# spyglass-search/memex

Hardware: AMD Instinct MI355X
Metric: queries/sec, exact cosine top-10 (recall@10 = 1.0) on 10M x 384-d f32 (higher is better)
Workload: dtype f32 corpus; int8 MFMA filter (exact integer sums, measured-residual certificate) -> f32 rescoring -> f64 DistCosine on the survivors (results bit-identical to all-f64)

## Files before the change

### memex_amd/csrc/index.hip

```cpp
#include <dlfcn.h>
#include <sys/stat.h>
#include <unistd.h>

#include <algorithm>
#include <atomic>
#include <cmath>
#include <condition_variable>
#include <cstdlib>
#include <chrono>
#include <ctime>
#include <cstring>
#include <deque>
#include <map>
#include <memory>
#include <mutex>
#include <string>
#include <thread>
#include <vector>

#include "index_kernels.h"
#include "mx_common.h"
#include "mx_debug.h"
#include "shard_pool.h"

// ... 124 lines not shown
    uint64_t plain_bf16_rows = 0;
    uint64_t demoted_at_rows = 0;
    float *tsc = nullptr;
    float *amean = nullptr;
    float *mean = nullptr;
    float *msum = nullptr;
    bool centred = false;
    bool compressed = false;
    bool raw_ingest = false;
    float *xs = nullptr, *ss = nullptr;
    uint64_t xs_rows = 0;
    uint64_t n = 0, cap = 0;
    IdMap idmap{0, 0, 1, 0};
    uint32_t *flags = nullptr;
    uint64_t wild_rows = 0;
    uint32_t *zero_rows = nullptr;
    uint64_t n_zero = 0;
    uint32_t *wild_list = nullptr;
    uint64_t n_wild = 0;
    int mode = MX_SEARCH_AUTO;
    bool profiling = false;
    int n_cu = 0, nwg = 0;
    bool scan8_pair = true;
    Scratch s;
    mx_index_stats stats{};
    hipEvent_t ev0 = nullptr, ev1 = nullptr, ev_wait = nullptr;
    double wait_ema_us[4] = {0.0, 0.0, 0.0, 0.0};
    uint64_t *dead = nullptr;
    std::vector<uint64_t> dead_h;
    uint64_t n_dead = 0;
    std::vector<uint64_t> dead_log;
    uint64_t disk_dead = 0;
    uint64_t gen = 0;
    bool failed = false;
    uint64_t *filt = nullptr;
    size_t filt_words = 0;
    uint64_t *filt_ranges = nullptr;
    size_t filt_ranges_cap = 0;
    uint32_t *subset_rows = nullptr;
    bool last_subset = false;
    std::string disk_dir;
    uint64_t disk_rows = 0;
    off_t disk_size = 0;
    struct timespec disk_mtime {};
    std::vector<mx_index *> shards;
    uint64_t block_rows = 0;
// ... 463 lines not shown
    idx->n += n;
    if (idx->filter_auto && idx->xh && !idx->filter_i8 && idx->demoted_at_rows && idx->n >= 2 * idx->demoted_at_rows &&
        idx->ds <= kAutoI8MaxDim) {
        const std::string keep = last_error_slot();
        if (build_filter_copy(idx, true) == MX_OK) {
            idx->demoted_at_rows = 0;
            idx->stats.filter_promotions += 1;
        } else {
            idx->demoted_at_rows = idx->n;
            last_error_slot() = keep;
        }
    }
    if (idx->xh && !idx->filter_i8 && !idx->compressed && !idx->centred && idx->kc <= kMaxKC && idx->n >= 256 &&
        idx->n >= 2 * std::max<uint64_t>(idx->plain_bf16_rows, 128) && !(idx->filter_auto && idx->demoted_at_rows)) {
        const std::string keep = last_error_slot();
        if (build_filter_copy(idx, false) != MX_OK) {
            idx->plain_bf16_rows = idx->n;
            last_error_slot() = keep;
        }
    }
    return MX_OK;
}

uint32_t sample_stride(uint64_t full_tiles, int nwg, int k, bool filt8, int ds, bool centred8 = false) {
    (void)centred8;
    double div = !filt8 ? 64.0 : ds <= 512 ? 16.0 : ds <= 768 ? 8.0 : 4.0;
    if (const int dv = debug_flag("sample_div", 0); dv >= 2 && dv <= 4096) div = (double)dv;
    const double f = std::min(0.5, std::max(1.0 / div, (double)k / 640.0));
    const uint64_t target = std::max<uint64_t>((uint64_t)nwg, (uint64_t)((double)full_tiles * f));
    return (uint32_t)std::max<uint64_t>(1, full_tiles / std::max<uint64_t>(target, 1));
}

constexpr size_t kExactKeepBytes = 256ull << 20;

int run_exact(mx_index *idx, const std::vector<int> &qs, int k, uint64_t *d_ids, float *d_scores, float *d_dists,
              int32_t *d_nfound, const uint64_t *mask, uint64_t n_live) {
    if (qs.empty()) return MX_OK;
    int gcap = qs.size() <= 4 ? 4 : qs.size() <= 8 ? 8 : qs.size() <= 16 ? 16 : kExactGroup;
    int rc = ensure_exact(idx, k, &gcap);
    if (rc != MX_OK) return rc;
    Scratch &s = idx->s;
    for (size_t g0 = 0; g0 < qs.size(); g0 += (size_t)gcap) {
        ExactGroup grp{};
        grp.n = (int)std::min<size_t>((size_t)gcap, qs.size() - g0);
        for (int j = 0; j < grp.n; ++j) grp.q[j] = qs[g0 + j];
        MX_HIP(launch_exact_group(idx->stream, k, idx->ds, idx->compressed ? nullptr : idx->x, idx->xh, idx->n, idx->idmap, s.qpad,
                                  s.qnorm2, grp, s.exact_scratch, d_ids, d_scores, d_dists, d_nfound, mask, n_live));
    }
    return MX_OK;
}

int build_filter_copy(mx_index *idx, bool i8) {
    DevBuf nh, nts, nec, nam;
// ... 326 lines not shown
        const uint64_t ts0 = filt ? fr.front().first / trows : 0, ts1 = filt ? (fr.back().second + trows - 1) / trows : tiles;
        const uint64_t full1 = std::min(ts1, full);
        ScanParams p;
        p.x = idx->x;
        p.xh = idx->xh;
        p.scale = idx->scale;
        p.qfrag = s.qfrag;
        p.theta = s.theta;
        p.n_rows = idx->n;
        p.ds = (uint32_t)idx->ds;
        p.wave_mask = (1u << ((B + 31) / 32)) - 1u;
        p.lane_rec = s.lane_rec;
        p.lane_tile = s.lane_tile;
        p.lane_cnt = s.lane_cnt;
        p.lane_max = s.lane_max;
        p.overflow = s.overflow;
        p.tscale = idx->tsc;
        p.qscale = s.qscale;
        p.qa = s.qa;
        p.qb = s.qb;
        p.amean = centred ? idx->amean : nullptr;
        p.qmean = s.qmean;
        p.dead = mask;
        auto scan = [&](bool collect) {
            if (filt8) return launch_scan8(st, idx->kc, collect, nwg, p, pair ? Scan8Geom::kPair : x2 ? Scan8Geom::k512 : Scan8Geom::k256);
            if (wide) return launch_scan16w(st, idx->kc, collect, idx->nwg, p);
            return idx->xh ? launch_scan16(st, idx->kc, collect, idx->nwg, p) : launch_scan(st, idx->kc, collect, idx->nwg, p);
        };
        auto collect = [&](bool first) -> int {
            p.tile_begin = (uint32_t)ts0;
            p.tile_end = (uint32_t)ts1;
            p.tile_stride = 1;
            if (first && idx->profiling) MX_HIP(hipEventRecord(idx->ev0, st));
            MX_HIP(scan(true));
            if (first && idx->profiling) {
                MX_HIP(hipEventRecord(idx->ev1, st));
                timed = true;
            }
            if (first) {
                idx->stats.scan_launches += 1;
                idx->stats.scan_bytes += (ts1 - ts0) * trows * idx->ds * (filt8 ? 1ull : idx->xh ? 2ull : 4ull);
            }
            return MX_OK;
        };
        if (ts1 - ts0 > 2ull * idx->nwg) {
            p.tile_begin = (uint32_t)ts0;
            p.tile_end = (uint32_t)full1;
            p.tile_stride = sample_stride(full1 - ts0, nwg, k, filt8, idx->ds, centred8);
            MX_HIP(scan(false));
            MX_HIP(launch_theta(st, B, k, nwg, s.lane_max, s.qa, !filt8, s.theta));
        }
        if ((rc = collect(true)) != MX_OK) return rc;
        if ((rc = finish_and_wait()) != MX_OK) return rc;
        if (timed) {
            float ms = 0.f;
            MX_HIP(hipEventElapsedTime(&ms, idx->ev0, idx->ev1));
            idx->stats.scan_ms += ms;
            timed = false;
        }
        if (s.host_sum[2]) return fail(MX_EINVAL, "a query contains non-finite values");
        idx->stats.candidates += s.host_sum[1];
        if (s.host_sum[0]) {
            if ((rc = fetch_flags()) != MX_OK) return rc;
            int retry = 0;
            for (int b = 0; b < B; ++b) {
                if (h_ovf[b] == 1) ++retry;
                else if (h_ovf[b] >= 2) exact.push_back(b);
            }
            if (filt8 && !filt) idx->i8_retry_batches += 1;
            const bool habitual = filt8 && idx->i8_batches >= 8 && idx->i8_retry_batches * 4 > idx->i8_batches;
            if (filt8 && !filt && idx->filter_auto && ((size_t)(retry + (int)exact.size()) * 16 > (size_t)std::max(B, 16) || habitual)) {
                if (!idx->centred && idx->kc <= kMaxKC && idx->n >= 256) {
// ... 1005 lines not shown
        if (g_scan_setup_err == hipSuccess) g_scan_setup_err = range_setup();
    });
    if (g_scan_setup_err != hipSuccess)
        return fail(MX_EDEVICE, "scan kernel setup failed: %s (is this a gfx950 device?)", hipGetErrorString(g_scan_setup_err));
    std::unique_ptr<mx_index> idx(new mx_index());
    idx->key = k;
    idx->dim = dim;
    idx->ds = (int)round_up((uint64_t)dim, dim > kMaxKC * kChunkFloats ? 2 * kChunkFloats : kChunkFloats);
    idx->kc = idx->ds / kChunkFloats;
    {
        const char *fk = getenv("MEMEX_HIP_FILTER");
        idx->filter_auto = !(fk && fk[0]);
        idx->filter_i8 = idx->filter_auto ? idx->ds <= kAutoI8MaxDim : (fk[0] == 'i' || fk[0] == '8');
    }
    idx->device = device;
    hipDeviceProp_t prop;
    MX_HIP(hipGetDeviceProperties(&prop, device));
    idx->n_cu = prop.multiProcessorCount;
    idx->nwg = std::max(1, std::min(idx->n_cu, kMaxScanCUs));
    {
        const char *pv = getenv("MEMEX_HIP_SCAN8_PAIR");
        idx->scan8_pair = !(pv && pv[0] == '0');
    }
    MX_HIP(hipStreamCreateWithFlags(&idx->stream, hipStreamNonBlocking));
    MX_HIP(hipEventCreate(&idx->ev0));
    MX_HIP(hipEventCreate(&idx->ev1));
    MX_HIP(hipEventCreateWithFlags(&idx->ev_wait, hipEventDisableTiming));
    MX_HIP(hipMalloc(&idx->flags, 6 * sizeof(uint32_t)));
    MX_HIP(hipMemset(idx->flags, 0, 6 * sizeof(uint32_t)));
    MX_HIP(hipMalloc(&idx->zero_rows, kZeroCap * sizeof(uint32_t)));
    MX_HIP(hipMalloc(&idx->wild_list, kWildCap * sizeof(uint32_t)));
    if (device < kMaxDevices) {
        std::lock_guard<std::mutex> lk(g_lanes[device].mu);
        g_lanes[device].open_indexes += 1;
        idx->pooled = true;
    }
    *out = idx.release();
    return MX_OK;
}

bool row_removed(const mx_index *t, uint64_t r) {
    return t->dead && (r >> 6) < t->dead_h.size() && ((t->dead_h[r >> 6] >> (r & 63)) & 1ull);
}
bool global_removed(const mx_index *idx, uint64_t r) {
    if (!idx->composite()) return row_removed(idx, r);
    const uint64_t R = idx->block_rows, G = idx->shards.size(), b = r / R;
// ... 181 lines not shown
    return release_capacity(idx);
}

int compact_composite(mx_index *idx) {
    const uint64_t R = idx->block_rows, G = idx->shards.size(), total = idx->total;
    std::unique_ptr<mx_index> fresh(new mx_index());
    fresh->dim = idx->dim;
    fresh->block_rows = R;
    auto drop_fresh = [&] {
        for (mx_index *sh : fresh->shards) free_index(sh);
        fresh->shards.clear();
    };
    for (uint64_t g = 0; g < G; ++g) {
        mx_index *old = idx->shards[g], *sh = nullptr;
        int rc = open_plain("", idx->dim, old->device, &sh);
        if (rc != MX_OK) {
            drop_fresh();
            return rc;
        }
        sh->idmap = old->idmap;
        sh->mode = old->mode;
        sh->profiling = old->profiling;
        sh->scan8_pair = old->scan8_pair;
        sh->want_filter = old->want_filter;
        sh->filter_i8 = old->filter_i8;
        sh->filter_auto = old->filter_auto;
        sh->compressed = old->compressed;
        sh->raw_ingest = old->compressed;
        fresh->shards.push_back(sh);
    }
    const uint64_t chunk = std::max<uint64_t>(kTile8Rows, (32ull << 20) / ((uint64_t)idx->dim * 4));
    std::vector<float> buf((size_t)std::min<uint64_t>(chunk, std::max<uint64_t>(total, 1)) * idx->dim), tmpv;
    int rc = MX_OK;
    for (uint64_t r0 = 0; r0 < total && rc == MX_OK; r0 += chunk) {
        const uint64_t m = std::min(chunk, total - r0);
        rc = fetch_rows(idx, r0, m, buf.data(), tmpv);
        uint64_t k = 0;
        for (uint64_t i = 0; i < m && rc == MX_OK; ++i) {
            if (global_removed(idx, r0 + i)) continue;
            if (k != i) memmove(buf.data() + k * idx->dim, buf.data() + i * idx->dim, (size_t)idx->dim * sizeof(float));
            ++k;
        }
        if (rc == MX_OK && k) rc = composite_add(fresh.get(), buf.data(), k, nullptr, false);
    }
    for (mx_index *sh : fresh->shards) sh->raw_ingest = false;
    if (rc != MX_OK) {
// ... 1119 lines not shown
```

### memex_amd/csrc/index_kernels.h

```cpp
#pragma once
#include <hip/hip_runtime.h>

#include <cstdint>

namespace mx {

constexpr int kScanThreads = 512;
constexpr int kScanWaves = 8;
constexpr int kTileRows = 32;
constexpr int kChunkFloats = 128;
constexpr int kSlotBytes = kTileRows * kChunkFloats * 4;
constexpr int kNumSlots = 8;
constexpr int kPrefetch = 8;
constexpr int kScaleRing = 16;
constexpr int kScanLdsBytes = kNumSlots * kSlotBytes + 2 * kTileRows * (kChunkFloats * 2 + 16) + kScaleRing * kTileRows * 4;
constexpr int kMaxKC = 6;

constexpr int kSlot16Bytes = kTileRows * kChunkFloats * 2;
constexpr int kRing16 = 16;
constexpr int kMeanRing16 = 32;
constexpr int kScan16LdsBytes = kRing16 * kSlot16Bytes + kMeanRing16 * 256 + 1024;
constexpr int kMaxKC16 = 12;
constexpr int kWideBatch = 128;
constexpr int kScan16WideLdsBytes = kRing16 * kSlot16Bytes + 4 * 64 * 16 * 4;
// ... 29 lines not shown
struct ScanParams {
    const float *x;
    const void *xh;
    const float *scale;
    const void *qfrag;
    const float *theta;
    uint64_t n_rows;
    uint32_t tile_begin;
    uint32_t tile_end;
    uint32_t tile_stride;
    uint32_t ds;
    uint32_t wave_mask = 0xff;
    float *lane_rec;
    uint32_t *lane_tile;
    uint32_t *lane_cnt;
    float *lane_max;
    uint32_t *overflow;
    const float *tscale = nullptr;
    const float *qscale = nullptr;
    const float *qa = nullptr, *qb = nullptr;
    const float *amean = nullptr;
    const float *qmean = nullptr;
    const uint64_t *dead = nullptr;
};

__device__ __forceinline__ uint32_t lane_dead16(uint32_t half, uint32_t h) {
    const uint32_t w = half >> (4u * h);
    return (w & 0xfu) | ((w >> 4) & 0xf0u) | ((w >> 8) & 0xf00u) | ((w >> 12) & 0xf000u);
}
__device__ __forceinline__ uint32_t dead_half(const uint64_t *dead, uint32_t t) { return (uint32_t)(dead[t >> 1] >> (32u * (t & 1u))); }

hipError_t scan_setup();
hipError_t scan16_setup();
hipError_t launch_scan(hipStream_t s, int kc, bool collect, int nwg, const ScanParams &p);
hipError_t launch_scan16(hipStream_t s, int kc, bool collect, int nwg, const ScanParams &p);
constexpr int kTile8Rows = 64;
constexpr int kTscaleFloats = 8;
constexpr float kMinStep8 = 1.0f / 32768.0f;
constexpr int kScaleRing8 = 32;
constexpr int kScale8Entry = 512;
constexpr int kScan8LdsBytes = kRing16 * kSlot16Bytes + kScaleRing8 * kScale8Entry + 256;
constexpr int kScan8PairWaves = 4;
constexpr int kScan8PairRing = 8;
constexpr int kScan8PairScaleRing = 16;
constexpr int kScan8PairEntry = 256;
constexpr int kScan8PairLdsBytes = kScan8PairRing * kSlot16Bytes + kScan8PairScaleRing * kScan8PairEntry;
static_assert(2 * kScan8PairLdsBytes <= 160 * 1024, "two workgroups of the pair form must fit one CU's LDS");
enum class Scan8Geom {
    k256,
    k512,
    kPair,
};
hipError_t scan8_setup();
hipError_t launch_scan8(hipStream_t s, int kc, bool collect, int nwg, const ScanParams &p, Scan8Geom geom = Scan8Geom::k256);
hipError_t launch_shadow8(hipStream_t s, const float *x, const float *scale, int ds, uint32_t half0, uint32_t half1,
                          uint64_t row_hi, void *x8, float *tscale, uint32_t *ec_max, const float *mean = nullptr,
                          float *amean = nullptr, uint32_t *rc_max = nullptr);
hipError_t scan16w_setup();
hipError_t launch_scan16w(hipStream_t s, int kc, bool collect, int nwg, const ScanParams &p);

hipError_t launch_shadow(hipStream_t s, const float *x, const float *scale, int ds, uint32_t tile0, uint32_t tile1,
                         void *xh, uint32_t *ec_max, uint32_t src_tile0 = 0, uint64_t row_lo = 0, uint64_t row_hi = ~0ull,
                         const float *mean = nullptr, float *amean = nullptr);
hipError_t launch_mean_dir(hipStream_t s, const float *x, const float *scale, uint64_t n, int ds, float *msum, float *mean);
hipError_t launch_unshadow(hipStream_t s, const void *xh, int ds, int d, uint64_t row0, uint64_t n, float *out);

hipError_t launch_ingest(hipStream_t s, const float *src, uint64_t n, int d, float *x, float *scale,
                         uint64_t first, int ds, uint32_t *flags, int raw, uint32_t *zero_rows, uint32_t *wild_rows, uint64_t row_base);

hipError_t launch_prep_queries(hipStream_t s, const float *q, int B, int d, int ds, void *qfrag,
                               float *qpad, double *qnorm2, float *theta, float *e1, const uint32_t *ec_max,
                               uint32_t *overflow, uint32_t *flags, float *qa, float *qb, bool filt8 = false,
                               float *qscale = nullptr, const float *mean = nullptr, float *qmean = nullptr,
                               const uint32_t *rc_max = nullptr);

hipError_t launch_theta(hipStream_t s, int B, int k, int nwg, const float *lane_max, const float *qa, bool raw, float *theta);

// ... 91 lines not shown
```

### memex_amd/csrc/index_kernels.hip

```cpp
#include <cmath>

#include "index_kernels.h"
#include "mx_rotate.h"

namespace mx {

typedef __attribute__((ext_vector_type(4))) float f32x4;

__device__ __forceinline__ uint32_t f32_key(float f) {
    const uint32_t u = __float_as_uint(f);
    return (u & 0x80000000u) ? ~u : (u | 0x80000000u);
}
__device__ __forceinline__ float key_f32(uint32_t k) {
    const uint32_t u = (k & 0x80000000u) ? (k & 0x7fffffffu) : ~k;
    return __uint_as_float(u);
}
__device__ __forceinline__ float score_from_dist(float d) {
    const float t = __fdiv_rn(1.0f, d);
    const float u = __fdiv_rn(1.0f, t);
    return __fsub_rn(1.0f, u);
}
__device__ __forceinline__ float dist_from_sums(double dot, double na, double nb) {
    if (na > 0.0 && nb > 0.0) {
        double d = __dsub_rn(1.0, __ddiv_rn(dot, __dsqrt_rn(__dmul_rn(na, nb))));
// ... 363 lines not shown
    const int n = 2 * nwg;
    const uint32_t t0 = (uint32_t)(q >> 5) * 64 + (uint32_t)(q & 31);
    uint32_t key[PER];
    bool valid[PER];
#pragma unroll
    for (int e = 0; e < PER; ++e) {
        const int i = e * 256 + tid;
        float v = -INFINITY;
        if (i < n) {
            const int hh = i / nwg, w = i - hh * nwg;
            v = lane_max[(size_t)(t0 + 32 * hh) * nwg + w];
        }
        valid[e] = v > -INFINITY;
        key[e] = f32_key(v);
    }
    uint32_t nv = 0;
#pragma unroll
    for (int e = 0; e < PER; ++e) nv += (uint32_t)__popcll(__builtin_amdgcn_ballot_w64(valid[e]));
    if ((tid & 63) == 0) s_nvalid[tid >> 6] = nv;
    __syncthreads();
    nv = s_nvalid[0] + s_nvalid[1] + s_nvalid[2] + s_nvalid[3];
    float kth = -8.0f;
    if (nv >= (uint32_t)k && k > 0) kth = key_f32(block_kth_largest<PER>(key, valid, (uint32_t)k, s_hist, s_pick));
    if (tid == 0 && theta[q] != INFINITY) theta[q] = kth - (raw ? 2.0f : 1.0f) * qa[q];
}

hipError_t launch_theta(hipStream_t s, int B, int k, int nwg, const float *lane_max, const float *qa, bool raw, float *theta) {
    if (B <= 0) return hipSuccess;
    if (nwg > kMaxScanWGs) return hipErrorInvalidValue;
    if (nwg <= 256)
        hipLaunchKernelGGL(theta_kernel<2>, dim3(B), dim3(256), 0, s, k, nwg, lane_max, qa, raw ? 1 : 0, theta);
    else
        hipLaunchKernelGGL(theta_kernel<4>, dim3(B), dim3(256), 0, s, k, nwg, lane_max, qa, raw ? 1 : 0, theta);
    return hipGetLastError();
}

__global__ void retry_setup_kernel(float *theta, const float *theta_retry, uint32_t *overflow, uint32_t *todo) {
    const int q = threadIdx.x;
    const bool again = overflow[q] == 1;
    todo[q] = again ? 1u : 0u;
    theta[q] = again ? theta_retry[q] : INFINITY;
    if (again) overflow[q] = 0;
}

hipError_t launch_retry_setup(hipStream_t s, float *theta, const float *theta_retry, uint32_t *overflow, uint32_t *todo) {
    hipLaunchKernelGGL(retry_setup_kernel, dim3(1), dim3(kMaxBatch), 0, s, theta, theta_retry, overflow, todo);
    return hipGetLastError();
// ... 1545 lines not shown
```

### memex_amd/csrc/scan8.hip

```cpp
#include <climits>
#include <type_traits>

#include "index_kernels.h"
#include "mx_rotate.h"

namespace mx {

typedef __attribute__((ext_vector_type(4))) int i32x4;
typedef __attribute__((ext_vector_type(16))) int i32x16;
typedef __attribute__((ext_vector_type(4))) float f32x4;
typedef __attribute__((address_space(3))) void lds_void;

#define MX_LDS_DMA16(rsrc, ldsptr, voff, soff, aux) \
    __builtin_amdgcn_raw_ptr_buffer_load_lds((rsrc), (lds_void *)(ldsptr), 16, (voff), (soff), 0, (aux))

#ifndef MX_SCAN8_ABLATE
#define MX_SCAN8_ABLATE 0
#endif

namespace {
template <int N>
using ic = std::integral_constant<int, N>;
template <int B, int E, class F>
__device__ __forceinline__ void static_for(F &&f) {
    if constexpr (B < E) {
        f(ic<B>{});
        static_for<B + 1, E>(f);
// ... 12 lines not shown

template <int KC, int MODE, int QG, bool CEN, int NW = kScanWaves, int RING = kRing16, bool DEAD = false>
__global__ __launch_bounds__(NW * 64, 2) void scan8_kernel(const ScanParams p) {
    static_assert(!CEN || (KC <= kMaxKC && QG == 1), "the centred form exists up to kMaxKC slots with one query group");
    static_assert((NW == kScanWaves && RING == kRing16) || (NW == kScan8PairWaves && RING == kScan8PairRing && QG == 2 && !CEN),
                  "one 8-wave workgroup with a 16-slot ring, or the two-workgroup form");
    static_assert((RING & (RING - 1)) == 0 && 8 % NW == 0, "");
    constexpr int DPS = 8 / NW;
    constexpr int TOPS = NW == kScanWaves ? 2 : 1;
    constexpr int SRING = NW == kScanWaves ? kScaleRing8 : kScan8PairScaleRing;
    constexpr int SENTRY = NW == kScanWaves ? kScale8Entry : kScan8PairEntry;
    constexpr uint32_t kSbase = RING * kSlot16Bytes;
    constexpr int R = QG == 2 ? (KC <= 3 ? 8 : 4) : KC <= 8 ? 8 : KC <= 10 ? 4 : 2;
    extern __shared__ __attribute__((aligned(16))) char smem[];
    constexpr bool centred = CEN;

    const int tid = threadIdx.x;
    const int lane = tid & 63;
    const int wave = __builtin_amdgcn_readfirstlane(tid >> 6);
    const int m = lane & 31;
    const bool live = KC == 12 || QG == 2 || ((p.wave_mask >> wave) & 1u) != 0;

    i32x4 qf[QG * KC * 4];
    float theta[QG], qa[QG], qb[QG], sq[QG];
    float aq = 0.0f;
#pragma unroll
    for (int g = 0; g < QG; ++g) {
        const int vw = wave * QG + g;
        const i32x4 *src = reinterpret_cast<const i32x4 *>(p.qfrag) + (size_t)vw * (KC * 4) * 64 + lane;
#pragma unroll
        for (int i = 0; i < KC * 4; ++i) qf[g * KC * 4 + i] = src[(size_t)i * 64];
        theta[g] = MODE == 1 ? p.theta[vw * 32 + m] : 0.0f;
        if (CEN && g == 0) aq = p.qmean[vw * 32 + m];
        qa[g] = MODE == 0 ? p.qa[vw * 32 + m] : 0.0f;
        qb[g] = p.qb[vw * 32 + m];
        sq[g] = p.qscale[vw * 32 + m];
    }
    const float kq = CEN && sq[0] > 0.0f ? aq / sq[0] : 0.0f;

    const uint32_t grid = gridDim.x;
    const uint32_t stride = p.tile_stride;
    const uint32_t t0 = p.tile_begin + blockIdx.x * stride;
    const uint32_t tstep = grid * stride;
    const uint32_t nT = (t0 < p.tile_end) ? (p.tile_end - t0 + tstep - 1) / tstep : 0;
    const uint32_t tilebytes = p.ds * (uint32_t)kTile8Rows;
    const uint32_t lane16 = (uint32_t)lane * 16u;
    const uint32_t lane4 = (uint32_t)lane * 4u;

    __amdgpu_buffer_rsrc_t rsrc;
    uint32_t is_ti = 0;
    auto tile_ops = [&](uint32_t it) {
        const uint32_t tile = t0 + it * tstep;
        const bool live_tile = it < nT;
        __amdgpu_buffer_rsrc_t srs = __builtin_amdgcn_make_buffer_rsrc((void *)(p.tscale + kTscaleFloats * (size_t)tile), 0, live_tile ? (uint32_t)(kTscaleFloats * 4) : 0u, 0x00020000);
        char *sdst = smem + __builtin_amdgcn_readfirstlane(kSbase + (it & (SRING - 1)) * SENTRY);
        __builtin_amdgcn_raw_ptr_buffer_load_lds(srs, (lds_void *)sdst, 4, lane4, 0, 0, 0);
        if constexpr (TOPS == 1) return;
        const float *abase = centred ? p.amean + (size_t)kTile8Rows * tile : p.tscale;
        const bool mine = live_tile && centred && (int)(it & 7u) == wave;
        __amdgpu_buffer_rsrc_t ars = __builtin_amdgcn_make_buffer_rsrc((void *)abase, 0, mine ? (uint32_t)(kTile8Rows * 4) : 0u, 0x00020000);
        char *adst = mine ? sdst + 256 : smem + kSbase + SRING * SENTRY;
        __builtin_amdgcn_raw_ptr_buffer_load_lds(ars, (lds_void *)adst, 4, lane4, 0, 0, 0);
    };
    auto open_tile = [&]() {
        const uint32_t tile = t0 + is_ti * tstep;
        const bool live_tile = is_ti < nT;
        tile_ops(is_ti + 1);
        const char *base = reinterpret_cast<const char *>(p.xh) + (size_t)tile * tilebytes;
        rsrc = __builtin_amdgcn_make_buffer_rsrc((void *)base, 0, live_tile ? tilebytes : 0u, 0x00020000);
        ++is_ti;
    };
    auto issue = [&](int kci, uint32_t ring_pos) {
        if (kci == 0) open_tile();
#pragma unroll
        for (int d = 0; d < DPS; ++d) {
            const int piece = wave + d * NW;
            char *dst = smem + __builtin_amdgcn_readfirstlane(ring_pos * kSlot16Bytes + piece * 1024);
            MX_LDS_DMA16(rsrc, dst, lane16, kci * kSlot16Bytes + piece * 1024, 2 );
        }
    };

    auto mylane = [&](int g) { return (uint32_t)((wave * QG + g) * 64 + lane) * gridDim.x + blockIdx.x; };
    uint32_t cnt[QG];
    float best[QG];
#pragma unroll
    for (int g = 0; g < QG; ++g) cnt[g] = 0, best[g] = -INFINITY;

    tile_ops(0);
#pragma unroll
    for (int i = 0; i < RING - 1; ++i) issue(i % KC, (uint32_t)i);

    i32x4 a[R];
    asm volatile("s_waitcnt vmcnt(%0)" ::"n"(ops_after<KC, DPS, TOPS>(1, RING - 2)) : "memory");
    __builtin_amdgcn_s_barrier();
#pragma unroll
    for (int f = 0; f < R; ++f) a[f] = *reinterpret_cast<const i32x4 *>(smem + lane16 + f * 1024);

    f32x4 shs_c = f32x4{0.0f, 0.0f, 0.0f, 0.0f};
    f32x4 shs_n = f32x4{0.0f, 0.0f, 0.0f, 0.0f};
    f32x4 inv_n = f32x4{0.0f, 0.0f, 0.0f, 0.0f};
    f32x4 acv[CEN ? 8 : 1];
    i32x16 init[CEN ? 2 : 1];
    i32x16 acc[QG * 2];
    auto entry_of = [&](uint32_t it) { return kSbase + (it & (SRING - 1)) * (uint32_t)SENTRY; };
    auto group_values = [&](int j) {
        const float ku = kq * ((j >> 2) ? inv_n[1] : inv_n[0]);
#pragma unroll
        for (int i = 0; i < 4; ++i) init[j >> 2][(j & 3) * 4 + i] = (int)(acv[j][i] * ku);
    };
    if constexpr (CEN) {
        if (live) {
            const uint32_t sa = entry_of(0), aa = sa + 256 + (lane >> 5) * 16;
            asm volatile("ds_read_b128 %0, %10\n\tds_read_b128 %1, %10 offset:16\n\t"
                         "ds_read_b128 %2, %11\n\tds_read_b128 %3, %11 offset:32\n\tds_read_b128 %4, %11 offset:64\n\tds_read_b128 %5, %11 offset:96\n\t"
                         "ds_read_b128 %6, %11 offset:128\n\tds_read_b128 %7, %11 offset:160\n\tds_read_b128 %8, %11 offset:192\n\tds_read_b128 %9, %11 offset:224\n\t"
                         "s_waitcnt lgkmcnt(0)"
                         : "=&v"(shs_c), "=&v"(inv_n), "=&v"(acv[0]), "=&v"(acv[1]), "=&v"(acv[2]), "=&v"(acv[3]), "=&v"(acv[4]), "=&v"(acv[5]),
                           "=&v"(acv[6]), "=&v"(acv[7])
                         : "v"(sa), "v"(aa)
                         : "memory");
#pragma unroll
            for (int j = 0; j < 8; ++j) group_values(j);
        }
    }
    uint32_t rp = 0;
#pragma unroll 1
    for (uint32_t ti = 0; ti < nT; ++ti) {
        const uint32_t tile = t0 + ti * tstep;
        uint64_t dw = 0;
        if constexpr (!CEN) {
#pragma unroll
            for (int g = 0; g < QG * 2; ++g)
#pragma unroll
                for (int r = 0; r < 16; ++r) acc[g][r] = 0;
        }

        static_for<0, KC>([&](auto kct) __attribute__((always_inline)) {
            constexpr int kc = decltype(kct)::value;
            const uint32_t rp1 = (rp + 1) & (RING - 1);
            const uint32_t rpi = (rp + RING - 1) & (RING - 1);
            if constexpr (DEAD && kc == 0) {
                asm volatile("s_load_dwordx2 %0, %1, 0x0\n\ts_waitcnt vmcnt(%2)\n\ts_barrier\n\ts_waitcnt lgkmcnt(0)"
                             : "=s"(dw)
                             : "s"(p.dead + tile), "n"(ops_after<KC, DPS, TOPS>(kc + 2, kc + RING - 2))
                             : "memory");
            } else {
                asm volatile("s_waitcnt vmcnt(%0)" ::"n"(ops_after<KC, DPS, TOPS>(kc + 2, kc + RING - 2)) : "memory");
                __builtin_amdgcn_s_barrier();
            }
            const uint32_t fb0 = rp * kSlot16Bytes + lane16, fb1 = rp1 * kSlot16Bytes + lane16;
            if (live) {
// ... 40 lines not shown
#endif
#pragma unroll
        for (int g = 0; g < QG; ++g) {
#pragma unroll
            for (int u = 0; u < 2; ++u) {
                i32x16 &ac = acc[g * 2 + u];
                const float sh = u ? shs[1] : shs[0], er = u ? shs[3] : shs[2];
                if constexpr (DEAD) {
                    const uint32_t hw = (uint32_t)(dw >> (32 * u));
                    if (hw) {
                        const uint32_t lb = lane_dead16(hw, (uint32_t)lane >> 5);
#pragma unroll
                        for (int r = 0; r < 16; ++r)
                            if ((lb >> r) & 1u) ac[r] = INT_MIN;
                    }
                }
                int mxi = max(max(ac[0], ac[1]), ac[2]);
#pragma unroll
                for (int r = 3; r < 15; r += 2) mxi = max(max(mxi, ac[r]), ac[r + 1]);
                mxi = max(mxi, ac[15]);
                float mx = ((float)mxi * sh) * sq[g];
                if (DEAD && mxi == INT_MIN) mx = -INFINITY;
                const float thr = fmaf(-qb[g], er, theta[g]);
                if (MODE == 0) {
                    best[g] = fmaxf(best[g], mx - fmaf(qb[g], er, qa[g]));
                } else if (__builtin_amdgcn_ballot_w64(mx >= thr) != 0) {
                    if (mx >= thr) {
                        if ((cnt[g] & 0x7fffffffu) < (uint32_t)kRecCap) {
                            const size_t at = (size_t)mylane(g) * kRecCap + (cnt[g] & 0x7fffffffu);
                            f32x4 *dst = reinterpret_cast<f32x4 *>(p.lane_rec + at * 16);
#pragma unroll
                            for (int i = 0; i < 4; ++i)
                                dst[i] = f32x4{((float)ac[4 * i] * sh) * sq[g], ((float)ac[4 * i + 1] * sh) * sq[g],
                                               ((float)ac[4 * i + 2] * sh) * sq[g], ((float)ac[4 * i + 3] * sh) * sq[g]};
                            p.lane_tile[at] = 2 * tile + u;
                            ++cnt[g];
                        } else {
                            cnt[g] |= 0x80000000u;
                        }
                    }
                }
            }
        }
        if constexpr (CEN) {
            asm volatile("s_waitcnt lgkmcnt(0)"
                         : "+v"(shs_n), "+v"(inv_n), "+v"(acv[0]), "+v"(acv[1]), "+v"(acv[2]), "+v"(acv[3]), "+v"(acv[4]), "+v"(acv[5]), "+v"(acv[6]), "+v"(acv[7])
                         :
                         : "memory");
#pragma unroll
            for (int j = 0; j < 8; ++j) group_values(j);
            shs_c = shs_n;
        }
    }
    asm volatile("s_waitcnt vmcnt(0)" ::: "memory");

#pragma unroll
    for (int g = 0; g < QG; ++g) {
        if (MODE == 0) {
            p.lane_max[mylane(g)] = best[g];
        } else {
            p.lane_cnt[mylane(g)] = cnt[g] & 0x7fffffffu;
            if (cnt[g] >> 31) p.overflow[(wave * QG + g) * 32 + m] = 1;
        }
    }
}

__global__ __launch_bounds__(256) void shadow8_kernel(const float *__restrict__ x, const float *__restrict__ scale, int ds,
                                                      uint32_t half0, uint32_t half1, uint64_t row_hi,
                                                      i32x4 *__restrict__ x8, float *__restrict__ tscale,
                                                      uint32_t *__restrict__ ec_max, const float *__restrict__ mean,
                                                      float *__restrict__ amean, uint32_t *__restrict__ rc_max) {
    extern __shared__ __attribute__((aligned(16))) char s8[];
    float *rbuf = reinterpret_cast<float *>(s8);
    int8_t *stage = reinterpret_cast<int8_t *>(s8 + (size_t)8 * ds * sizeof(float));
    float *mix = reinterpret_cast<float *>(s8 + (size_t)8 * ds * sizeof(float) + (size_t)kTileRows * ds);
    float *s_r2 = mix + kRotMaxBlocks * kRotMaxBlocks;
    float *s_red = s_r2 + kTileRows;
    float *s_ac = s_red + 4;
    const int tid = threadIdx.x, lane = tid & 63, wave = tid >> 6;
    const int kc = ds >> 7;
    const uint32_t frags = (uint32_t)(ds >> 5) * 64u;
    float *in = rbuf + (size_t)wave * 2 * ds, *out = in + ds;
    rot_fill_mix(mix, kc, tid, 256);
// ... 109 lines not shown
                               hipFuncAttributeMaxDynamicSharedMemorySize, kScan8LdsBytes);
}
template <int KC, int MODE>
static hipError_t setup8_pair() {
    hipError_t e = hipFuncSetAttribute(reinterpret_cast<const void *>(&scan8_kernel<KC, MODE, 2, false, kScan8PairWaves, kScan8PairRing>),
                                       hipFuncAttributeMaxDynamicSharedMemorySize, kScan8PairLdsBytes);
    if (e != hipSuccess) return e;
    return hipFuncSetAttribute(reinterpret_cast<const void *>(&scan8_kernel<KC, MODE, 2, false, kScan8PairWaves, kScan8PairRing, true>),
                               hipFuncAttributeMaxDynamicSharedMemorySize, kScan8PairLdsBytes);
}

hipError_t scan8_setup() {
    hipError_t e;
    if ((e = hipFuncSetAttribute(reinterpret_cast<const void *>(&shadow8_kernel), hipFuncAttributeMaxDynamicSharedMemorySize,
                                 (int)shadow8_lds(kMaxKC16 * kChunkFloats))) != hipSuccess)
        return e;
#define MX_SETUP(KC)                                             \
    if ((e = setup8_one<KC, 0, 1>()) != hipSuccess) return e;    \
    if ((e = setup8_one<KC, 1, 1>()) != hipSuccess) return e;
    MX_SETUP(1) MX_SETUP(2) MX_SETUP(3) MX_SETUP(4) MX_SETUP(5) MX_SETUP(6)
    MX_SETUP(7) MX_SETUP(8) MX_SETUP(9) MX_SETUP(10) MX_SETUP(11) MX_SETUP(12)
#undef MX_SETUP
#define MX_SETUP(KC)                                             \
    if ((e = setup8_one<KC, 0, 2>()) != hipSuccess) return e;    \
    if ((e = setup8_one<KC, 1, 2>()) != hipSuccess) return e;
    MX_SETUP(1) MX_SETUP(2) MX_SETUP(3) MX_SETUP(4)
#undef MX_SETUP
#define MX_SETUP(KC)                                             \
    if ((e = setup8_pair<KC, 0>()) != hipSuccess) return e;      \
    if ((e = setup8_pair<KC, 1>()) != hipSuccess) return e;
    MX_SETUP(1) MX_SETUP(2) MX_SETUP(3) MX_SETUP(4)
#undef MX_SETUP
#define MX_SETUP(KC)                                                   \
    if ((e = setup8_one<KC, 0, 1, true>()) != hipSuccess) return e;    \
    if ((e = setup8_one<KC, 1, 1, true>()) != hipSuccess) return e;
    MX_SETUP(1) MX_SETUP(2) MX_SETUP(3) MX_SETUP(4) MX_SETUP(5) MX_SETUP(6)
#undef MX_SETUP
    static_assert(kMaxKC == 6, "one centred scan8_kernel per slot count up to kMaxKC");
    return hipSuccess;
}

template <int KC, int QG, bool CEN = false>
static hipError_t launch8_kc(hipStream_t s, bool collect, int nwg, const ScanParams &p) {
    if (p.dead) {
        if (collect) hipLaunchKernelGGL((scan8_kernel<KC, 1, QG, CEN, kScanWaves, kRing16, true>), dim3(nwg), dim3(kScanThreads), kScan8LdsBytes, s, p);
        else hipLaunchKernelGGL((scan8_kernel<KC, 0, QG, CEN, kScanWaves, kRing16, true>), dim3(nwg), dim3(kScanThreads), kScan8LdsBytes, s, p);
        return hipGetLastError();
    }
    if (collect)
        hipLaunchKernelGGL((scan8_kernel<KC, 1, QG, CEN>), dim3(nwg), dim3(kScanThreads), kScan8LdsBytes, s, p);
    else
        hipLaunchKernelGGL((scan8_kernel<KC, 0, QG, CEN>), dim3(nwg), dim3(kScanThreads), kScan8LdsBytes, s, p);
    return hipGetLastError();
}

template <int KC>
static hipError_t launch8_pair(hipStream_t s, bool collect, int nwg, const ScanParams &p) {
    constexpr int NW = kScan8PairWaves, RING = kScan8PairRing;
    if (p.dead) {
        if (collect) hipLaunchKernelGGL((scan8_kernel<KC, 1, 2, false, NW, RING, true>), dim3(nwg), dim3(NW * 64), kScan8PairLdsBytes, s, p);
        else hipLaunchKernelGGL((scan8_kernel<KC, 0, 2, false, NW, RING, true>), dim3(nwg), dim3(NW * 64), kScan8PairLdsBytes, s, p);
        return hipGetLastError();
    }
    if (collect)
        hipLaunchKernelGGL((scan8_kernel<KC, 1, 2, false, NW, RING>), dim3(nwg), dim3(NW * 64), kScan8PairLdsBytes, s, p);
    else
        hipLaunchKernelGGL((scan8_kernel<KC, 0, 2, false, NW, RING>), dim3(nwg), dim3(NW * 64), kScan8PairLdsBytes, s, p);
    return hipGetLastError();
}

hipError_t launch_scan8(hipStream_t s, int kc, bool collect, int nwg, const ScanParams &p, Scan8Geom geom) {
    if (geom == Scan8Geom::kPair) {
        if (p.amean) return hipErrorInvalidValue;
        switch (kc) {
            case 1: return launch8_pair<1>(s, collect, nwg, p);
            case 2: return launch8_pair<2>(s, collect, nwg, p);
            case 3: return launch8_pair<3>(s, collect, nwg, p);
            case 4: return launch8_pair<4>(s, collect, nwg, p);
            default: return hipErrorInvalidValue;
        }
    }
    if (geom == Scan8Geom::k512) {
        if (p.amean) return hipErrorInvalidValue;
        switch (kc) {
            case 1: return launch8_kc<1, 2>(s, collect, nwg, p);
            case 2: return launch8_kc<2, 2>(s, collect, nwg, p);
            case 3: return launch8_kc<3, 2>(s, collect, nwg, p);
            case 4: return launch8_kc<4, 2>(s, collect, nwg, p);
            default: return hipErrorInvalidValue;
        }
    }
    if (p.amean) {
        switch (kc) {
            case 1: return launch8_kc<1, 1, true>(s, collect, nwg, p);
            case 2: return launch8_kc<2, 1, true>(s, collect, nwg, p);
            case 3: return launch8_kc<3, 1, true>(s, collect, nwg, p);
            case 4: return launch8_kc<4, 1, true>(s, collect, nwg, p);
            case 5: return launch8_kc<5, 1, true>(s, collect, nwg, p);
            case 6: return launch8_kc<6, 1, true>(s, collect, nwg, p);
            default: return hipErrorInvalidValue;
        }
    }
    switch (kc) {
        case 1: return launch8_kc<1, 1>(s, collect, nwg, p);
        case 2: return launch8_kc<2, 1>(s, collect, nwg, p);
        case 3: return launch8_kc<3, 1>(s, collect, nwg, p);
        case 4: return launch8_kc<4, 1>(s, collect, nwg, p);
        case 5: return launch8_kc<5, 1>(s, collect, nwg, p);
        case 6: return launch8_kc<6, 1>(s, collect, nwg, p);
        case 7: return launch8_kc<7, 1>(s, collect, nwg, p);
        case 8: return launch8_kc<8, 1>(s, collect, nwg, p);
        case 9: return launch8_kc<9, 1>(s, collect, nwg, p);
        case 10: return launch8_kc<10, 1>(s, collect, nwg, p);
        case 11: return launch8_kc<11, 1>(s, collect, nwg, p);
        case 12: return launch8_kc<12, 1>(s, collect, nwg, p);
        default: return hipErrorInvalidValue;
    }
}

}
```

Measured before the change: 234,700.

## Collect during threshold sampling and skip sampled tiles in the full scan

The int8 threshold-sampling pass now runs in three stages. A sparse presample sets an initial theta, then a denser sample pass (mode 2) both tracks per-lane maxima and records candidates above that theta. The final collect scan (mode 3) then walks a SkipMap that skips the tiles already covered by the sample, using a stride chosen to divide the workgroup count. This removes the double read of sampled tiles and allows a denser sample (divisor 8 instead of 16 for ds<=512), which should tighten theta. The cost is an extra small launch, more kernel instantiations and more complex tile indexing. theta is now updated monotonically with fmaxf.

```diff
diff --git a/memex_amd/csrc/index.hip b/memex_amd/csrc/index.hip
--- a/memex_amd/csrc/index.hip
+++ b/memex_amd/csrc/index.hip
@@ -170,6 +170,7 @@
     bool profiling = false;
     int n_cu = 0, nwg = 0;
     bool scan8_pair = true;
+    bool sample_skip = true;
     Scratch s;
     mx_index_stats stats{};
     hipEvent_t ev0 = nullptr, ev1 = nullptr, ev_wait = nullptr;
@@ -679,13 +680,20 @@
     return MX_OK;
 }
 
-uint32_t sample_stride(uint64_t full_tiles, int nwg, int k, bool filt8, int ds, bool centred8 = false) {
+uint32_t sample_stride(uint64_t full_tiles, int nwg, int k, bool filt8, int ds, bool centred8 = false, bool skip8 = false) {
     (void)centred8;
-    double div = !filt8 ? 64.0 : ds <= 512 ? 16.0 : ds <= 768 ? 8.0 : 4.0;
+    double div = !filt8 ? 64.0 : ds <= 512 ? (skip8 ? 8.0 : 16.0) : ds <= 768 ? 8.0 : 4.0;
     if (const int dv = debug_flag("sample_div", 0); dv >= 2 && dv <= 4096) div = (double)dv;
     const double f = std::min(0.5, std::max(1.0 / div, (double)k / 640.0));
     const uint64_t target = std::max<uint64_t>((uint64_t)nwg, (uint64_t)((double)full_tiles * f));
     return (uint32_t)std::max<uint64_t>(1, full_tiles / std::max<uint64_t>(target, 1));
+}
+
+constexpr uint32_t kPreSample = 16;
+uint32_t skip_stride(uint32_t stride, uint32_t nwg) {
+    for (uint32_t s = stride; s >= 2; --s)
+        if (nwg % s == 0) return s;
+    return 0;
 }
 
 constexpr size_t kExactKeepBytes = 256ull << 20;
@@ -1058,32 +1066,48 @@
         p.amean = centred ? idx->amean : nullptr;
         p.qmean = s.qmean;
         p.dead = mask;
-        auto scan = [&](bool collect) {
-            if (filt8) return launch_scan8(st, idx->kc, collect, nwg, p, pair ? Scan8Geom::kPair : x2 ? Scan8Geom::k512 : Scan8Geom::k256);
+        auto scan = [&](int mode) {
+            if (filt8) return launch_scan8(st, idx->kc, mode, nwg, p, pair ? Scan8Geom::kPair : x2 ? Scan8Geom::k512 : Scan8Geom::k256);
+            const bool collect = mode != 0;
             if (wide) return launch_scan16w(st, idx->kc, collect, idx->nwg, p);
             return idx->xh ? launch_scan16(st, idx->kc, collect, idx->nwg, p) : launch_scan(st, idx->kc, collect, idx->nwg, p);
         };
+        uint32_t skip = 0;
         auto collect = [&](bool first) -> int {
             p.tile_begin = (uint32_t)ts0;
             p.tile_end = (uint32_t)ts1;
             p.tile_stride = 1;
+            p.skip_stride = first ? skip : 0u;
+            p.skip_end = (uint32_t)full1;
             if (first && idx->profiling) MX_HIP(hipEventRecord(idx->ev0, st));
-            MX_HIP(scan(true));
+            MX_HIP(scan(1));
             if (first && idx->profiling) {
                 MX_HIP(hipEventRecord(idx->ev1, st));
                 timed = true;
             }
             if (first) {
+                const uint64_t sampled = p.skip_stride ? (full1 - ts0 + p.skip_stride - 1) / p.skip_stride : 0;
                 idx->stats.scan_launches += 1;
-                idx->stats.scan_bytes += (ts1 - ts0) * trows * idx->ds * (filt8 ? 1ull : idx->xh ? 2ull : 4ull);
+                idx->stats.scan_bytes += (ts1 - ts0 - sampled) * trows * idx->ds * (filt8 ? 1ull : idx->xh ? 2ull : 4ull);
             }
             return MX_OK;
         };
         if (ts1 - ts0 > 2ull * idx->nwg) {
             p.tile_begin = (uint32_t)ts0;
             p.tile_end = (uint32_t)full1;
-            p.tile_stride = sample_stride(full1 - ts0, nwg, k, filt8, idx->ds, centred8);
-            MX_HIP(scan(false));
+            const bool skip8 = filt8 && !centred8 && idx->sample_skip && idx->kc <= kMaxKC8x2;
+            p.tile_stride = sample_stride(full1 - ts0, nwg, k, filt8, idx->ds, centred8, skip8);
+            if (skip8) skip = skip_stride(p.tile_stride, (uint32_t)nwg);
+            if (skip) {
+                const int pre = debug_flag("presample", (int)kPreSample);
+                p.tile_stride = skip * (uint32_t)std::min(std::max(pre, 1), 256);
+                MX_HIP(scan(0));
+                MX_HIP(launch_theta(st, B, k, nwg, s.lane_max, s.qa, false, s.theta));
+                p.tile_stride = skip;
+                MX_HIP(scan(2));
+            } else {
+                MX_HIP(scan(0));
+            }
             MX_HIP(launch_theta(st, B, k, nwg, s.lane_max, s.qa, !filt8, s.theta));
         }
         if ((rc = collect(true)) != MX_OK) return rc;
@@ -2135,6 +2159,10 @@
         const char *pv = getenv("MEMEX_HIP_SCAN8_PAIR");
         idx->scan8_pair = !(pv && pv[0] == '0');
     }
+    {
+        const char *pv = getenv("MEMEX_HIP_SAMPLE_SKIP");
+        idx->sample_skip = !(pv && pv[0] == '0');
+    }
     MX_HIP(hipStreamCreateWithFlags(&idx->stream, hipStreamNonBlocking));
     MX_HIP(hipEventCreate(&idx->ev0));
     MX_HIP(hipEventCreate(&idx->ev1));
@@ -2362,6 +2390,7 @@
         sh->mode = old->mode;
         sh->profiling = old->profiling;
         sh->scan8_pair = old->scan8_pair;
+        sh->sample_skip = old->sample_skip;
         sh->want_filter = old->want_filter;
         sh->filter_i8 = old->filter_i8;
         sh->filter_auto = old->filter_auto;
diff --git a/memex_amd/csrc/index_kernels.h b/memex_amd/csrc/index_kernels.h
--- a/memex_amd/csrc/index_kernels.h
+++ b/memex_amd/csrc/index_kernels.h
@@ -75,6 +75,8 @@
     const float *amean = nullptr;
     const float *qmean = nullptr;
     const uint64_t *dead = nullptr;
+    uint32_t skip_stride = 0;
+    uint32_t skip_end = 0;
 };
 
 __device__ __forceinline__ uint32_t lane_dead16(uint32_t half, uint32_t h) {
@@ -105,7 +107,7 @@
     kPair,
 };
 hipError_t scan8_setup();
-hipError_t launch_scan8(hipStream_t s, int kc, bool collect, int nwg, const ScanParams &p, Scan8Geom geom = Scan8Geom::k256);
+hipError_t launch_scan8(hipStream_t s, int kc, int mode, int nwg, const ScanParams &p, Scan8Geom geom = Scan8Geom::k256);
 hipError_t launch_shadow8(hipStream_t s, const float *x, const float *scale, int ds, uint32_t half0, uint32_t half1,
                           uint64_t row_hi, void *x8, float *tscale, uint32_t *ec_max, const float *mean = nullptr,
                           float *amean = nullptr, uint32_t *rc_max = nullptr);
diff --git a/memex_amd/csrc/index_kernels.hip b/memex_amd/csrc/index_kernels.hip
--- a/memex_amd/csrc/index_kernels.hip
+++ b/memex_amd/csrc/index_kernels.hip
@@ -409,7 +409,7 @@
     nv = s_nvalid[0] + s_nvalid[1] + s_nvalid[2] + s_nvalid[3];
     float kth = -8.0f;
     if (nv >= (uint32_t)k && k > 0) kth = key_f32(block_kth_largest<PER>(key, valid, (uint32_t)k, s_hist, s_pick));
-    if (tid == 0 && theta[q] != INFINITY) theta[q] = kth - (raw ? 2.0f : 1.0f) * qa[q];
+    if (tid == 0 && theta[q] != INFINITY) theta[q] = fmaxf(theta[q], kth - (raw ? 2.0f : 1.0f) * qa[q]);
 }
 
 hipError_t launch_theta(hipStream_t s, int B, int k, int nwg, const float *lane_max, const float *qa, bool raw, float *theta) {
diff --git a/memex_amd/csrc/mx_skipmap.h b/memex_amd/csrc/mx_skipmap.h
--- /dev/null
+++ b/memex_amd/csrc/mx_skipmap.h
@@ -0,0 +1,55 @@
+#pragma once
+#include <cstdint>
+
+#if defined(__HIPCC__)
+#define MX_SKIPMAP_HD __host__ __device__ __forceinline__
+#else
+#define MX_SKIPMAP_HD inline
+#endif
+
+namespace mx {
+
+struct SkipMap {
+    uint32_t w, grid, S, c;
+    uint32_t begin, skip_end;
+    uint32_t nrot;
+    uint32_t n;
+
+    MX_SKIPMAP_HD SkipMap(uint32_t w_, uint32_t grid_, uint32_t S_, uint32_t begin_, uint32_t skip_end_, uint32_t end_)
+        : w(w_), grid(grid_), S(S_), c(w_ % S_), begin(begin_), skip_end(skip_end_) {
+        const uint32_t nf = skip_end - begin, r0 = nf / grid, rem = nf - r0 * grid;
+        nrot = r0 - (r0 + S - 1 - c) / S;
+        if (r0 % S != c && slot(r0) < rem) ++nrot;
+        const uint32_t nt = end_ - skip_end;
+        n = nrot + (w < nt ? (nt - w + grid - 1) / grid : 0u);
+    }
+    MX_SKIPMAP_HD uint32_t slot(uint32_t i) const { return c ? w : w + i % S; }
+    MX_SKIPMAP_HD uint32_t tile(uint32_t it) const {
+        if (it < nrot) {
+            const uint32_t i = it + (it + S - 1 - c) / (S - 1);
+            return begin + i * grid + slot(i);
+        }
+        return skip_end + w + (it - nrot) * grid;
+    }
+    struct Cursor {
+        uint32_t it, i, im;
+    };
+    MX_SKIPMAP_HD Cursor first() const {
+        const uint32_t i0 = c == 0 ? 1u : 0u;
+        return Cursor{0u, i0, i0 % S};
+    }
+    MX_SKIPMAP_HD uint32_t tile(const Cursor &k) const {
+        return k.it < nrot ? begin + k.i * grid + (c ? w : w + k.im) : skip_end + w + (k.it - nrot) * grid;
+    }
+    MX_SKIPMAP_HD void next(Cursor &k) const {
+        ++k.it;
+        ++k.i;
+        k.im = k.im + 1 == S ? 0u : k.im + 1;
+        if (k.im == c) {
+            ++k.i;
+            k.im = k.im + 1 == S ? 0u : k.im + 1;
+        }
+    }
+};
+
+}
diff --git a/memex_amd/csrc/scan8.hip b/memex_amd/csrc/scan8.hip
--- a/memex_amd/csrc/scan8.hip
+++ b/memex_amd/csrc/scan8.hip
@@ -3,6 +3,7 @@
 
 #include "index_kernels.h"
 #include "mx_rotate.h"
+#include "mx_skipmap.h"
 
 namespace mx {
 
@@ -61,6 +62,7 @@
     const bool live = KC == 12 || QG == 2 || ((p.wave_mask >> wave) & 1u) != 0;
 
     i32x4 qf[QG * KC * 4];
+    constexpr bool kMax = MODE == 0 || MODE == 2, kRec = MODE != 0, kSkip = MODE == 3;
     float theta[QG], qa[QG], qb[QG], sq[QG];
     float aq = 0.0f;
 #pragma unroll
@@ -69,9 +71,9 @@
         const i32x4 *src = reinterpret_cast<const i32x4 *>(p.qfrag) + (size_t)vw * (KC * 4) * 64 + lane;
 #pragma unroll
         for (int i = 0; i < KC * 4; ++i) qf[g * KC * 4 + i] = src[(size_t)i * 64];
-        theta[g] = MODE == 1 ? p.theta[vw * 32 + m] : 0.0f;
+        theta[g] = MODE != 0 ? p.theta[vw * 32 + m] : 0.0f;
         if (CEN && g == 0) aq = p.qmean[vw * 32 + m];
-        qa[g] = MODE == 0 ? p.qa[vw * 32 + m] : 0.0f;
+        qa[g] = kMax ? p.qa[vw * 32 + m] : 0.0f;
         qb[g] = p.qb[vw * 32 + m];
         sq[g] = p.qscale[vw * 32 + m];
     }
@@ -81,7 +83,15 @@
     const uint32_t stride = p.tile_stride;
     const uint32_t t0 = p.tile_begin + blockIdx.x * stride;
     const uint32_t tstep = grid * stride;
-    const uint32_t nT = (t0 < p.tile_end) ? (p.tile_end - t0 + tstep - 1) / tstep : 0;
+    const SkipMap smap(blockIdx.x, grid, kSkip ? p.skip_stride : 1u, p.tile_begin, kSkip ? p.skip_end : p.tile_begin, p.tile_end);
+    const uint32_t nT = kSkip ? smap.n : (t0 < p.tile_end) ? (p.tile_end - t0 + tstep - 1) / tstep : 0;
+    SkipMap::Cursor walk_ops = smap.first(), walk_dma = walk_ops, walk_epi = walk_ops;
+    auto tile_at = [&](uint32_t it, SkipMap::Cursor &k) {
+        if constexpr (!kSkip) return t0 + it * tstep;
+        const uint32_t t = smap.tile(k);
+        smap.next(k);
+        return t;
+    };
     const uint32_t tilebytes = p.ds * (uint32_t)kTile8Rows;
     const uint32_t lane16 = (uint32_t)lane * 16u;
     const uint32_t lane4 = (uint32_t)lane * 4u;
@@ -89,7 +99,7 @@
     __amdgpu_buffer_rsrc_t rsrc;
     uint32_t is_ti = 0;
     auto tile_ops = [&](uint32_t it) {
-        const uint32_t tile = t0 + it * tstep;
+        const uint32_t tile = tile_at(it, walk_ops);
         const bool live_tile = it < nT;
         __amdgpu_buffer_rsrc_t srs = __builtin_amdgcn_make_buffer_rsrc((void *)(p.tscale + kTscaleFloats * (size_t)tile), 0, live_tile ? (uint32_t)(kTscaleFloats * 4) : 0u, 0x00020000);
         char *sdst = smem + __builtin_amdgcn_readfirstlane(kSbase + (it & (SRING - 1)) * SENTRY);
@@ -102,7 +112,7 @@
         __builtin_amdgcn_raw_ptr_buffer_load_lds(ars, (lds_void *)adst, 4, lane4, 0, 0, 0);
     };
     auto open_tile = [&]() {
-        const uint32_t tile = t0 + is_ti * tstep;
+        const uint32_t tile = tile_at(is_ti, walk_dma);
         const bool live_tile = is_ti < nT;
         tile_ops(is_ti + 1);
         const char *base = reinterpret_cast<const char *>(p.xh) + (size_t)tile * tilebytes;
@@ -123,7 +133,7 @@
     uint32_t cnt[QG];
     float best[QG];
 #pragma unroll
-    for (int g = 0; g < QG; ++g) cnt[g] = 0, best[g] = -INFINITY;
+    for (int g = 0; g < QG; ++g) cnt[g] = kSkip ? p.lane_cnt[mylane(g)] : 0u, best[g] = -INFINITY;
 
     tile_ops(0);
 #pragma unroll
@@ -165,7 +175,7 @@
     uint32_t rp = 0;
 #pragma unroll 1
     for (uint32_t ti = 0; ti < nT; ++ti) {
-        const uint32_t tile = t0 + ti * tstep;
+        const uint32_t tile = tile_at(ti, walk_epi);
         uint64_t dw = 0;
         if constexpr (!CEN) {
 #pragma unroll
@@ -252,9 +262,8 @@
                 float mx = ((float)mxi * sh) * sq[g];
                 if (DEAD && mxi == INT_MIN) mx = -INFINITY;
                 const float thr = fmaf(-qb[g], er, theta[g]);
-                if (MODE == 0) {
-                    best[g] = fmaxf(best[g], mx - fmaf(qb[g], er, qa[g]));
-                } else if (__builtin_amdgcn_ballot_w64(mx >= thr) != 0) {
+                if (kMax) best[g] = fmaxf(best[g], mx - fmaf(qb[g], er, qa[g]));
+                if (kRec && __builtin_amdgcn_ballot_w64(mx >= thr) != 0) {
                     if (mx >= thr) {
                         if ((cnt[g] & 0x7fffffffu) < (uint32_t)kRecCap) {
                             const size_t at = (size_t)mylane(g) * kRecCap + (cnt[g] & 0x7fffffffu);
@@ -286,9 +295,8 @@
 
 #pragma unroll
     for (int g = 0; g < QG; ++g) {
-        if (MODE == 0) {
-            p.lane_max[mylane(g)] = best[g];
-        } else {
+        if (kMax) p.lane_max[mylane(g)] = best[g];
+        if (kRec) {
             p.lane_cnt[mylane(g)] = cnt[g] & 0x7fffffffu;
             if (cnt[g] >> 31) p.overflow[(wave * QG + g) * 32 + m] = 1;
         }
@@ -444,13 +452,22 @@
     MX_SETUP(7) MX_SETUP(8) MX_SETUP(9) MX_SETUP(10) MX_SETUP(11) MX_SETUP(12)
 #undef MX_SETUP
 #define MX_SETUP(KC)                                             \
+    if ((e = setup8_one<KC, 2, 1>()) != hipSuccess) return e;    \
+    if ((e = setup8_one<KC, 3, 1>()) != hipSuccess) return e;
+    MX_SETUP(1) MX_SETUP(2) MX_SETUP(3) MX_SETUP(4)
+#undef MX_SETUP
+#define MX_SETUP(KC)                                             \
     if ((e = setup8_one<KC, 0, 2>()) != hipSuccess) return e;    \
-    if ((e = setup8_one<KC, 1, 2>()) != hipSuccess) return e;
+    if ((e = setup8_one<KC, 1, 2>()) != hipSuccess) return e;    \
+    if ((e = setup8_one<KC, 2, 2>()) != hipSuccess) return e;    \
+    if ((e = setup8_one<KC, 3, 2>()) != hipSuccess) return e;
     MX_SETUP(1) MX_SETUP(2) MX_SETUP(3) MX_SETUP(4)
 #undef MX_SETUP
 #define MX_SETUP(KC)                                             \
     if ((e = setup8_pair<KC, 0>()) != hipSuccess) return e;      \
-    if ((e = setup8_pair<KC, 1>()) != hipSuccess) return e;
+    if ((e = setup8_pair<KC, 1>()) != hipSuccess) return e;      \
+    if ((e = setup8_pair<KC, 2>()) != hipSuccess) return e;      \
+    if ((e = setup8_pair<KC, 3>()) != hipSuccess) return e;
     MX_SETUP(1) MX_SETUP(2) MX_SETUP(3) MX_SETUP(4)
 #undef MX_SETUP
 #define MX_SETUP(KC)                                                   \
@@ -462,80 +479,85 @@
     return hipSuccess;
 }
 
+template <int KC, int QG, bool CEN, int NW, int RING, bool DEAD>
+static hipError_t launch8_mode(hipStream_t s, int mode, int nwg, int threads, int lds, const ScanParams &p) {
+    if (mode == 1 && p.skip_stride) mode = 3;
+    switch (mode) {
+        case 0: hipLaunchKernelGGL((scan8_kernel<KC, 0, QG, CEN, NW, RING, DEAD>), dim3(nwg), dim3(threads), lds, s, p); break;
+        case 1: hipLaunchKernelGGL((scan8_kernel<KC, 1, QG, CEN, NW, RING, DEAD>), dim3(nwg), dim3(threads), lds, s, p); break;
+        case 2:
+            if constexpr (CEN || KC > kMaxKC8x2) return hipErrorInvalidValue;
+            else hipLaunchKernelGGL((scan8_kernel<KC, 2, QG, CEN, NW, RING, DEAD>), dim3(nwg), dim3(threads), lds, s, p);
+            break;
+        case 3:
+            if constexpr (CEN || KC > kMaxKC8x2) return hipErrorInvalidValue;
+            else hipLaunchKernelGGL((scan8_kernel<KC, 3, QG, CEN, NW, RING, DEAD>), dim3(nwg), dim3(threads), lds, s, p);
+            break;
+        default: return hipErrorInvalidValue;
+    }
+    return hipGetLastError();
+}
+
 template <int KC, int QG, bool CEN = false>
-static hipError_t launch8_kc(hipStream_t s, bool collect, int nwg, const ScanParams &p) {
-    if (p.dead) {
-        if (collect) hipLaunchKernelGGL((scan8_kernel<KC, 1, QG, CEN, kScanWaves, kRing16, true>), dim3(nwg), dim3(kScanThreads), kScan8LdsBytes, s, p);
-        else hipLaunchKernelGGL((scan8_kernel<KC, 0, QG, CEN, kScanWaves, kRing16, true>), dim3(nwg), dim3(kScanThreads), kScan8LdsBytes, s, p);
-        return hipGetLastError();
-    }
-    if (collect)
-        hipLaunchKernelGGL((scan8_kernel<KC, 1, QG, CEN>), dim3(nwg), dim3(kScanThreads), kScan8LdsBytes, s, p);
-    else
-        hipLaunchKernelGGL((scan8_kernel<KC, 0, QG, CEN>), dim3(nwg), dim3(kScanThreads), kScan8LdsBytes, s, p);
-    return hipGetLastError();
+static hipError_t launch8_kc(hipStream_t s, int mode, int nwg, const ScanParams &p) {
+    if (p.dead) return launch8_mode<KC, QG, CEN, kScanWaves, kRing16, true>(s, mode, nwg, kScanThreads, kScan8LdsBytes, p);
+    return launch8_mode<KC, QG, CEN, kScanWaves, kRing16, false>(s, mode, nwg, kScanThreads, kScan8LdsBytes, p);
 }
 
 template <int KC>
-static hipError_t launch8_pair(hipStream_t s, bool collect, int nwg, const ScanParams &p) {
+static hipError_t launch8_pair(hipStream_t s, int mode, int nwg, const ScanParams &p) {
     constexpr int NW = kScan8PairWaves, RING = kScan8PairRing;
-    if (p.dead) {
-        if (collect) hipLaunchKernelGGL((scan8_kernel<KC, 1, 2, false, NW, RING, true>), dim3(nwg), dim3(NW * 64), kScan8PairLdsBytes, s, p);
-        else hipLaunchKernelGGL((scan8_kernel<KC, 0, 2, false, NW, RING, true>), dim3(nwg), dim3(NW * 64), kScan8PairLdsBytes, s, p);
-        return hipGetLastError();
-    }
-    if (collect)
-        hipLaunchKernelGGL((scan8_kernel<KC, 1, 2, false, NW, RING>), dim3(nwg), dim3(NW * 64), kScan8PairLdsBytes, s, p);
-    else
-        hipLaunchKernelGGL((scan8_kernel<KC, 0, 2, false, NW, RING>), dim3(nwg), dim3(NW * 64), kScan8PairLdsBytes, s, p);
-    return hipGetLastError();
-}
-
-hipError_t launch_scan8(hipStream_t s, int kc, bool collect, int nwg, const ScanParams &p, Scan8Geom geom) {
+    if (p.dead) return launch8_mode<KC, 2, false, NW, RING, true>(s, mode, nwg, NW * 64, kScan8PairLdsBytes, p);
+    return launch8_mode<KC, 2, false, NW, RING, false>(s, mode, nwg, NW * 64, kScan8PairLdsBytes, p);
+}
+
+hipError_t launch_scan8(hipStream_t s, int kc, int mode, int nwg, const ScanParams &p, Scan8Geom geom) {
+    if (p.skip_stride && (mode != 1 || kc > kMaxKC8x2 || p.skip_stride < 2 || nwg % p.skip_stride || p.skip_end < p.tile_begin || p.skip_end > p.tile_end))
+        return hipErrorInvalidValue;
     if (geom == Scan8Geom::kPair) {
         if (p.amean) return hipErrorInvalidValue;
         switch (kc) {
-            case 1: return launch8_pair<1>(s, collect, nwg, p);
-            case 2: return launch8_pair<2>(s, collect, nwg, p);
-            case 3: return launch8_pair<3>(s, collect, nwg, p);
-            case 4: return launch8_pair<4>(s, collect, nwg, p);
+            case 1: return launch8_pair<1>(s, mode, nwg, p);
+            case 2: return launch8_pair<2>(s, mode, nwg, p);
+            case 3: return launch8_pair<3>(s, mode, nwg, p);
+            case 4: return launch8_pair<4>(s, mode, nwg, p);
             default: return hipErrorInvalidValue;
         }
     }
     if (geom == Scan8Geom::k512) {
         if (p.amean) return hipErrorInvalidValue;
         switch (kc) {
-            case 1: return launch8_kc<1, 2>(s, collect, nwg, p);
-            case 2: return launch8_kc<2, 2>(s, collect, nwg, p);
-            case 3: return launch8_kc<3, 2>(s, collect, nwg, p);
-            case 4: return launch8_kc<4, 2>(s, collect, nwg, p);
+            case 1: return launch8_kc<1, 2>(s, mode, nwg, p);
+            case 2: return launch8_kc<2, 2>(s, mode, nwg, p);
+            case 3: return launch8_kc<3, 2>(s, mode, nwg, p);
+            case 4: return launch8_kc<4, 2>(s, mode, nwg, p);
             default: return hipErrorInvalidValue;
         }
     }
     if (p.amean) {
         switch (kc) {
-            case 1: return launch8_kc<1, 1, true>(s, collect, nwg, p);
-            case 2: return launch8_kc<2, 1, true>(s, collect, nwg, p);
-            case 3: return launch8_kc<3, 1, true>(s, collect, nwg, p);
-            case 4: return launch8_kc<4, 1, true>(s, collect, nwg, p);
-            case 5: return launch8_kc<5, 1, true>(s, collect, nwg, p);
-            case 6: return launch8_kc<6, 1, true>(s, collect, nwg, p);
+            case 1: return launch8_kc<1, 1, true>(s, mode, nwg, p);
+            case 2: return launch8_kc<2, 1, true>(s, mode, nwg, p);
+            case 3: return launch8_kc<3, 1, true>(s, mode, nwg, p);
+            case 4: return launch8_kc<4, 1, true>(s, mode, nwg, p);
+            case 5: return launch8_kc<5, 1, true>(s, mode, nwg, p);
+            case 6: return launch8_kc<6, 1, true>(s, mode, nwg, p);
             default: return hipErrorInvalidValue;
         }
     }
     switch (kc) {
-        case 1: return launch8_kc<1, 1>(s, collect, nwg, p);
-        case 2: return launch8_kc<2, 1>(s, collect, nwg, p);
-        case 3: return launch8_kc<3, 1>(s, collect, nwg, p);
-        case 4: return launch8_kc<4, 1>(s, collect, nwg, p);
-        case 5: return launch8_kc<5, 1>(s, collect, nwg, p);
-        case 6: return launch8_kc<6, 1>(s, collect, nwg, p);
-        case 7: return launch8_kc<7, 1>(s, collect, nwg, p);
-        case 8: return launch8_kc<8, 1>(s, collect, nwg, p);
-        case 9: return launch8_kc<9, 1>(s, collect, nwg, p);
-        case 10: return launch8_kc<10, 1>(s, collect, nwg, p);
-        case 11: return launch8_kc<11, 1>(s, collect, nwg, p);
-        case 12: return launch8_kc<12, 1>(s, collect, nwg, p);
+        case 1: return launch8_kc<1, 1>(s, mode, nwg, p);
+        case 2: return launch8_kc<2, 1>(s, mode, nwg, p);
+        case 3: return launch8_kc<3, 1>(s, mode, nwg, p);
+        case 4: return launch8_kc<4, 1>(s, mode, nwg, p);
+        case 5: return launch8_kc<5, 1>(s, mode, nwg, p);
+        case 6: return launch8_kc<6, 1>(s, mode, nwg, p);
+        case 7: return launch8_kc<7, 1>(s, mode, nwg, p);
+        case 8: return launch8_kc<8, 1>(s, mode, nwg, p);
+        case 9: return launch8_kc<9, 1>(s, mode, nwg, p);
+        case 10: return launch8_kc<10, 1>(s, mode, nwg, p);
+        case 11: return launch8_kc<11, 1>(s, mode, nwg, p);
+        case 12: return launch8_kc<12, 1>(s, mode, nwg, p);
         default: return hipErrorInvalidValue;
     }
 }
```

Measured after the change: 239,100, median of 6. +1.9%, better.
